# kobejean/nerf-qa

Hardware: AMD Instinct MI355X
Metric: DISTS frame-pairs/s (higher is better)
Workload: dtype f16

## Files before the change

nerf_qa_amd/csrc/nqa_conv.hip:

```cpp

#include "nqa_common.h"
#include "nqa_regw.h"

namespace nqa {

template <typename P>
__global__ __launch_bounds__(256) void conv1_1_kernel(const float *__restrict__ x, const float *__restrict__ w,
                                                      const float *__restrict__ bias,
                                                      typename P::T *__restrict__ out, int H, int W) {
  typedef typename P::T T;
  constexpr int HC = 128 / (int)sizeof(T);
  constexpr int PITCH = 128 + 16;
  __shared__ __attribute__((aligned(16))) char tile[256 * PITCH];
  const int HW = H * W;
  const int tid = threadIdx.x;
  const int pix0 = blockIdx.x * 256, pix = pix0 + tid;
  const int n = blockIdx.y;
  const bool live = pix < HW;
  const int py = live ? pix / W : 0, px = live ? pix - py * W : 0;
  float in[27];
  const float *xi = x + (size_t)n * 3 * HW;
#pragma unroll
  for (int ky = 0; ky < 3; ++ky) {
#pragma unroll
// ... 19 lines not shown
      f32x2 acc2[8];
#pragma unroll
      for (int j = 0; j < 8; ++j) acc2[j] = *reinterpret_cast<const f32x2 *>(bias + c0 + 2 * j);
#pragma unroll
      for (int k = 0; k < 27; ++k) {
#pragma unroll
        for (int j = 0; j < 8; ++j)
          acc2[j] = in[k] * *reinterpret_cast<const f32x2 *>(w + k * 64 + c0 + 2 * j) + acc2[j];
      }
      float acc[16];
#pragma unroll
      for (int j = 0; j < 16; ++j) acc[j] = acc2[j >> 1][j & 1];
      T *row = reinterpret_cast<T *>(tile + tid * PITCH) + g * 16;
      if constexpr (P::SPLIT) {
#pragma unroll
        for (int j = 0; j < 16; j += 4)
          store_split4(reinterpret_cast<char *>(row), j, fmaxf(acc[j], 0.f), fmaxf(acc[j + 1], 0.f),
                       fmaxf(acc[j + 2], 0.f), fmaxf(acc[j + 3], 0.f));
      } else if constexpr (sizeof(T) == 4) {
#pragma unroll
        for (int j = 0; j < 16; j += 4) {
          f32x4 v = {fmaxf(acc[j], 0.f), fmaxf(acc[j + 1], 0.f), fmaxf(acc[j + 2], 0.f), fmaxf(acc[j + 3], 0.f)};
          *reinterpret_cast<f32x4 *>(row + j) = v;
        }
      } else {
        typedef __attribute__((ext_vector_type(8))) T t8;
#pragma unroll
        for (int j = 0; j < 16; j += 8) {
          t8 v;
#pragma unroll
          for (int e = 0; e < 8; ++e) v[e] = P::from_f(fmaxf(acc[j + e], 0.f));
          *reinterpret_cast<t8 *>(row + j) = v;
        }
      }
    }
    __syncthreads();
#pragma unroll
    for (int r = 0; r < 8; ++r) {
      const int i = r * 256 + tid, p = i >> 3, ch = i & 7;
      if (p < npix)
        *reinterpret_cast<u32x4 *>(o + (size_t)p * 64 * sizeof(T) + half * 128 + ch * 16) =
            *reinterpret_cast<const u32x4 *>(tile + p * PITCH + ch * 16);
    }
    if (half + 1 < 64 / HC) __syncthreads();
  }
}


#ifdef NQA_STAMPS
__device__ unsigned long long g_stamps[8];
__device__ inline unsigned long long stamp() {
  unsigned long long t;
  __builtin_amdgcn_sched_barrier(0);
  asm volatile("s_memtime %0\n\ts_waitcnt lgkmcnt(0)" : "=s"(t)::"memory");
  __builtin_amdgcn_sched_barrier(0);
  return t;
}
#define NQA_STAMP(var) const unsigned long long var = stamp()
#define NQA_STAMP_ADD(seg, a, b) seg_sum[seg] += (b) - (a)
#else
#define NQA_STAMP(var)
#define NQA_STAMP_ADD(seg, a, b)
#endif

template <int WAVES_N, int WAVES_M, int WN_T, int WM_T, int TW, bool PAD8 = false>
struct ConvGeom {
  static constexpr int THREADS = 64 * WAVES_N * WAVES_M;
  static constexpr int BN = WAVES_N * WN_T * 32;
  static constexpr int NSUB = BN / 64;
  static constexpr int MP = WAVES_M * WM_T * 32;
  static constexpr int TH = MP / TW;
  static constexpr int HW_ = TW + 2, HH_ = TH + 2;
  static constexpr int HP = PAD8 ? (HW_ + 7) / 8 * 8 : HW_;
  static constexpr int NQ = HP * HH_;
  static constexpr int A_ITEMS = NQ * 4;
  static constexpr int A_ITEMS_PAD = (A_ITEMS + 63) / 64 * 64;
  static constexpr int A_BYTES = A_ITEMS_PAD * 16;
  static constexpr int A_ROUNDS = (A_ITEMS_PAD + THREADS - 1) / THREADS;
  static constexpr int SUB_STAGE_ITEMS = 3 * 64 * 4;
  static constexpr int W_ITEMS = NSUB * SUB_STAGE_ITEMS;
  static constexpr int W_BYTES = W_ITEMS * 16;
  static constexpr int W_ROUNDS = W_ITEMS / THREADS;
  static constexpr int LDS_BYTES = 2 * (A_BYTES + W_BYTES);
  static_assert(BN % 64 == 0 && W_ITEMS % THREADS == 0 && MP % TW == 0, "bad conv geometry");
};
static_assert(ConvGeom<2, 4, 4, 2, 32, true>::LDS_BYTES == 149504 && ConvGeom<2, 4, 4, 2, 16, true>::LDS_BYTES == 153600 &&
                  ConvGeom<2, 4, 2, 4, 32, true>::LDS_BYTES <= 163840,
              "8-wave M16 tiles: LDS budget");
static_assert(ConvGeom<2, 2, 2, 2, 32, true>::LDS_BYTES == 79872 && ConvGeom<2, 2, 2, 2, 16, true>::LDS_BYTES == 79872 &&
                  2 * 79872 <= 163840,
              "4-wave M16 tiles must keep two blocks per CU");

template <typename P, int WAVES_N, int WAVES_M, int WN_T, int WM_T, int TW, bool M16, int NTERM = 1, bool LOACC = false>
__device__ __forceinline__ void conv3x3_igemm_tile(
    const typename P::T *in, const char *wpk, const float *bias, typename P::T *out, int H, int W, int Cin, int Cout,
    int out_split, float floor_v, const int n, const int x0, const int y0, const int ct, char *const smem) {
#if defined(__HIP_DEVICE_COMPILE__)
  typedef typename P::T T;
  typedef ConvGeom<WAVES_N, WAVES_M, WN_T, WM_T, TW, M16> G;

  const int tid = threadIdx.x, lane = tid & 63;
  const int wave = __builtin_amdgcn_readfirstlane(tid >> 6);
  const int l31 = lane & 31, h = lane >> 5;
#if !defined(NQA_PRIO_SPLIT)
#define NQA_PRIO_SPLIT 2
#endif
  if (NQA_PRIO_SPLIT && M16 && WAVES_N * WAVES_M == 8 && wave >= 4) __builtin_amdgcn_s_setprio(NQA_PRIO_SPLIT);
  const int wn = wave % WAVES_N, wm = wave / WAVES_N;
  const int nCC = Cin / P::KC;
  const int S = nCC * 3 * NTERM;

  unsigned a_goff[G::A_ROUNDS];
#pragma unroll
  for (int r = 0; r < G::A_ROUNDS; ++r) {
    const int i = r * G::THREADS + tid;
    const int q = i >> 2, c = (i & 3) ^ lds_swz<M16>(q);
    const int hy = q / G::HP, hx = q - hy * G::HP;
    const int gy = y0 - 1 + hy, gx = x0 - 1 + hx;
    const bool ok = i < G::A_ITEMS && hx < G::HW_ && (unsigned)gy < (unsigned)H && (unsigned)gx < (unsigned)W;
    a_goff[r] = ok ? (unsigned)(((gy * W + gx) * Cin + c * P::CPC) * (int)sizeof(T)) : kOOB;
    if (!ok && i < G::A_ITEMS_PAD) {
      const u32x4 z = {0u, 0u, 0u, 0u};
      *reinterpret_cast<u32x4 *>(smem + i * 16) = z;
      *reinterpret_cast<u32x4 *>(smem + G::A_BYTES + i * 16) = z;
    }
  }
  const unsigned img_bytes = (unsigned)H * (unsigned)W * (unsigned)Cin * (unsigned)sizeof(T);
  const __amdgpu_buffer_rsrc_t a_rsrc = __builtin_amdgcn_make_buffer_rsrc(
      const_cast<T *>(in + (size_t)n * H * W * Cin), 0, img_bytes, 0x00020000);
  const unsigned sub_stride = (unsigned)nCC * 9u * 64u * 64u * (unsigned)NTERM;
  const __amdgpu_buffer_rsrc_t w_rsrc = __builtin_amdgcn_make_buffer_rsrc(
      const_cast<char *>(wpk + (size_t)ct * G::NSUB * sub_stride), 0, G::NSUB * sub_stride, 0x00020000);
  unsigned w_goff[G::W_ROUNDS];
#pragma unroll
  for (int r = 0; r < G::W_ROUNDS; ++r) {
    const int i = r * G::THREADS + tid;
    w_goff[r] = (unsigned)(i / G::SUB_STAGE_ITEMS) * sub_stride + (unsigned)(i % G::SUB_STAGE_ITEMS) * 16u;
  }
  const int wave_base = wave * 64 * 16;

  auto issue = [&](int s, int cc, bool first) {
#ifndef NQA_ABLATE_NO_DMA
    char *wdst = smem + 2 * G::A_BYTES + (s & 1) * G::W_BYTES + wave_base;
#pragma unroll
    for (int r = 0; r < G::W_ROUNDS; ++r)
      __builtin_amdgcn_raw_ptr_buffer_load_lds(w_rsrc, (lds_void_t *)(wdst + r * G::THREADS * 16), 16, w_goff[r],
                                               s * (G::SUB_STAGE_ITEMS * 16), 0, 0);
    if (first) {
      char *adst = smem + (cc & 1) * G::A_BYTES + wave_base;
#pragma unroll
      for (int r = 0; r < G::A_ROUNDS; ++r) {
        if (r * G::THREADS + wave * 64 < G::A_ITEMS_PAD)
          __builtin_amdgcn_raw_ptr_buffer_load_lds(a_rsrc, (lds_void_t *)(adst + r * G::THREADS * 16), 16, a_goff[r],
                                                   cc * 64, 0, 0);
      }
    }
#endif
  };
  auto dma_wait = [] { asm volatile("s_waitcnt vmcnt(0)" ::: "memory"); };

  int w_base[WN_T], w_sw[WN_T];
#pragma unroll
  for (int i = 0; i < WN_T; ++i) {
    const int cib = (wn * WN_T + i) * 32 + l31;
    const int r64 = cib & 63;
    w_base[i] = 2 * G::A_BYTES + (cib >> 6) * (G::SUB_STAGE_ITEMS * 16) + r64 * 64;
    w_sw[i] = (r64 >> 2) & 3;
  }
  int q0[WM_T];
#pragma unroll
  for (int j = 0; j < WM_T; ++j) {
    const int m = (wm * WM_T + j) * 32 + l31;
    const int ty = m / TW, tx = m - ty * TW;
    q0[j] = ty * G::HW_ + tx;
  }

  f32x16 acc[WN_T][WM_T];
#pragma unroll
  for (int i = 0; i < WN_T; ++i)
#pragma unroll
    for (int j = 0; j < WM_T; ++j)
#pragma unroll
      for (int r = 0; r < 16; ++r) acc[i][j][r] = 0.f;
  static_assert(!LOACC || (P::SPLIT && !M16), "LOACC: the split-f16 products only");
  f32x16 acc_lo[LOACC ? WN_T : 1][LOACC ? WM_T : 1];
  if constexpr (LOACC) {
#pragma unroll
    for (int i = 0; i < WN_T; ++i)
#pragma unroll
      for (int j = 0; j < WM_T; ++j)
#pragma unroll
        for (int r = 0; r < 16; ++r) acc_lo[i][j][r] = 0.f;
  }
  const int l15 = lane & 15, c4 = lane >> 4;
  int w16_base = 0, a16_base[3] = {0, 0, 0};
  auto w16_off = [](int i) { return (i >> 2) * (G::SUB_STAGE_ITEMS * 16) + (i & 3) * 1024; };
  auto a16_off = [](int j) { return ((j * 16 / TW) * G::HP + j * 16 % TW) * 64; };
  f32x4 acc16[2 * WN_T][2 * WM_T];
  if constexpr (M16) {
    static_assert(WN_T % 2 == 0 && (TW == 16 || TW == 32) && G::HP % 8 == 0 && (WM_T * 32) % TW == 0,
                  "the M16 loop's constant fragment offsets");
    static_assert(((2 * WM_T - 1) * 16 / TW * G::HP + 16) * 64 < 65536 &&
                      ((2 * WN_T - 1) >> 2) * (G::SUB_STAGE_ITEMS * 16) + 3 * 1024 + 2 * 4096 < 65536,
                  "an M16 fragment offset does not fit a ds_read immediate");
    w16_base = 2 * G::A_BYTES + wn * (WN_T / 2) * (G::SUB_STAGE_ITEMS * 16) + l15 * 64 + ((c4 ^ lds_swz<true>(l15)) << 4);
    const int qb = (wm * WM_T * 32 / TW) * G::HP + l15;
#pragma unroll
    for (int kx = 0; kx < 3; ++kx) a16_base[kx] = (qb + kx) * 64 + ((c4 ^ lds_swz<true>(qb + kx)) << 4);
#pragma unroll
    for (int i = 0; i < 2 * WN_T; ++i)
#pragma unroll
      for (int j = 0; j < 2 * WM_T; ++j) acc16[i][j] = (f32x4){0.f, 0.f, 0.f, 0.f};
  }

#ifdef NQA_STAMPS
  unsigned long long seg_sum[4] = {0, 0, 0, 0};
#endif
  issue(0, 0, true);
  for (int s = 0, cc = 0, sub = 0; s < S; ++s) {
    const int ky = sub / NTERM;
    const int sub_next = sub + 1 == 3 * NTERM ? 0 : sub + 1, cc_next = sub_next ? cc : cc + 1;
    NQA_STAMP(t0);
    dma_wait();
    NQA_STAMP(t1);
    __syncthreads();
    NQA_STAMP(t2);
    if (s + 1 < S) issue(s + 1, cc_next, sub_next == 0);
    NQA_STAMP(t3);
    NQA_STAMP_ADD(0, t0, t1);
    NQA_STAMP_ADD(1, t1, t2);
    NQA_STAMP_ADD(2, t2, t3);
    const char *abuf = smem + (cc & 1) * G::A_BYTES;
    const char *wbuf = smem + (s & 1) * G::W_BYTES;
    auto load_frags = [&](int t, u32x4(&af)[WN_T], u32x4(&bf)[WM_T]) {
      const int kx = t >> 1, ch = 2 * (t & 1) + h;
#pragma unroll
      for (int i = 0; i < WN_T; ++i)
        af[i] = *reinterpret_cast<const u32x4 *>(wbuf + w_base[i] + kx * 4096 + ((ch ^ w_sw[i]) << 4));
#pragma unroll
      for (int j = 0; j < WM_T; ++j) {
        const int q = q0[j] + ky * G::HW_ + kx;
        bf[j] = *reinterpret_cast<const u32x4 *>(abuf + q * 64 + ((ch ^ ((q >> 2) & 3)) << 4));
      }
    };
    auto mma_all = [&](const u32x4(&af)[WN_T], const u32x4(&bf)[WM_T]) {
#ifndef NQA_ABLATE_NO_MFMA
#pragma unroll
      for (int i = 0; i < WN_T; ++i)
#pragma unroll
        for (int j = 0; j < WM_T; ++j) acc[i][j] = P::mma(af[i], bf[j], acc[i][j]);
#else
#pragma unroll
      for (int i = 0; i < WN_T; ++i) asm volatile("" ::"v"(af[i]));
#pragma unroll
      for (int j = 0; j < WM_T; ++j) asm volatile("" ::"v"(bf[j]));
#endif
    };
    if constexpr (M16) {
      u32x4 af[2][WN_T], bf[2][2 * WM_T];
      const int a_stage = (cc & 1) * G::A_BYTES + ky * (G::HP * 64);
      const char *const wst = smem + (w16_base + (s & 1) * G::W_BYTES);
      const char *const ast[3] = {smem + (a16_base[0] + a_stage), smem + (a16_base[1] + a_stage),
                                  smem + (a16_base[2] + a_stage)};
      auto load16 = [&](int t) {
        const int kx = t >> 1, half = t & 1;
#pragma unroll
        for (int i = 0; i < WN_T; ++i)
          af[t & 1][i] = *reinterpret_cast<const u32x4 *>(wst + (w16_off(half * WN_T + i) + kx * 4096));
        if (half == 0) {
#pragma unroll
          for (int j = 0; j < 2 * WM_T; ++j) bf[kx & 1][j] = *reinterpret_cast<const u32x4 *>(ast[kx] + a16_off(j));
        }
      };
      auto mma16 = [&](int t) {
        const int kx = t >> 1, half = t & 1;
#pragma unroll
        for (int i = 0; i < WN_T; ++i)
#pragma unroll
          for (int j = 0; j < 2 * WM_T; ++j) {
            f32x4 &c = acc16[half * WN_T + i][j];
            c = P::mma16(af[t & 1][i], bf[kx & 1][j], c);
          }
      };
      load16(0);
#pragma unroll
      for (int t = 0; t < 6; ++t) {
        if (t + 1 < 6) load16(t + 1);
        __builtin_amdgcn_sched_barrier(0);
        mma16(t);
        __builtin_amdgcn_sched_barrier(0);
      }
    } else if constexpr (P::SPLIT) {
      auto load_split = [&](int kx, u32x4(&ah)[WN_T], u32x4(&al)[WN_T], u32x4(&bh)[WM_T], u32x4(&bl)[WM_T]) {
#pragma unroll
        for (int i = 0; i < WN_T; ++i) {
          const char *row = wbuf + w_base[i] + kx * 4096;
          ah[i] = *reinterpret_cast<const u32x4 *>(row + ((h ^ w_sw[i]) << 4));
          al[i] = *reinterpret_cast<const u32x4 *>(row + (((2 + h) ^ w_sw[i]) << 4));
        }
#pragma unroll
        for (int j = 0; j < WM_T; ++j) {
          const int q = q0[j] + ky * G::HW_ + kx, sw = (q >> 2) & 3;
          bh[j] = *reinterpret_cast<const u32x4 *>(abuf + q * 64 + ((h ^ sw) << 4));
          bl[j] = *reinterpret_cast<const u32x4 *>(abuf + q * 64 + (((2 + h) ^ sw) << 4));
        }
      };
      auto mma_split = [&](const u32x4(&ah)[WN_T], const u32x4(&al)[WN_T], const u32x4(&bh)[WM_T],
                           const u32x4(&bl)[WM_T]) {
#pragma unroll
        for (int term = 0; term < 3; ++term)
#pragma unroll
          for (int i = 0; i < WN_T; ++i)
#pragma unroll
            for (int j = 0; j < WM_T; ++j) {
              f32x16 &c = (LOACC && term < 2) ? acc_lo[LOACC ? i : 0][LOACC ? j : 0] : acc[i][j];
              c = __builtin_amdgcn_mfma_f32_32x32x16_f16(__builtin_bit_cast(f16x8, term == 0 ? al[i] : ah[i]),
                                                         __builtin_bit_cast(f16x8, term == 1 ? bl[j] : bh[j]), c, 0, 0, 0);
            }
      };
      u32x4 ahA[WN_T], alA[WN_T], bhA[WM_T], blA[WM_T], ahB[WN_T], alB[WN_T], bhB[WM_T], blB[WM_T];
      load_split(0, ahA, alA, bhA, blA);
      load_split(1, ahB, alB, bhB, blB);
      __builtin_amdgcn_sched_barrier(0);
      mma_split(ahA, alA, bhA, blA);
      __builtin_amdgcn_sched_barrier(0);
      load_split(2, ahA, alA, bhA, blA);
      __builtin_amdgcn_sched_barrier(0);
      mma_split(ahB, alB, bhB, blB);
      __builtin_amdgcn_sched_barrier(0);
      mma_split(ahA, alA, bhA, blA);
      __builtin_amdgcn_sched_barrier(0);
    } else {
    u32x4 afA[WN_T], bfA[WM_T], afB[WN_T], bfB[WM_T];
    load_frags(0, afA, bfA);
#pragma unroll
    for (int t = 0; t < 6; t += 2) {
      load_frags(t + 1, afB, bfB);
      __builtin_amdgcn_sched_barrier(0);
      mma_all(afA, bfA);
      __builtin_amdgcn_sched_barrier(0);
      if (t + 2 < 6) load_frags(t + 2, afA, bfA);
      __builtin_amdgcn_sched_barrier(0);
      mma_all(afB, bfB);
      __builtin_amdgcn_sched_barrier(0);
    }
    }
    NQA_STAMP(t4);
    NQA_STAMP_ADD(3, t3, t4);
    cc = cc_next;
    sub = sub_next;
  }
#ifdef NQA_STAMPS
  if (lane == 0) {
    for (int i = 0; i < 4; ++i) atomicAdd(&g_stamps[i], seg_sum[i]);
    atomicAdd(&g_stamps[4], (unsigned long long)S);
  }
#endif

  if constexpr (LOACC) {
#pragma unroll
    for (int i = 0; i < WN_T; ++i)
#pragma unroll
      for (int j = 0; j < WM_T; ++j) acc[i][j] += acc_lo[i][j];
  }
  constexpr int RB = G::BN * (int)sizeof(T), NCH = RB / 16, SWZ = NCH >= 16 ? 15 : NCH - 1;
  constexpr int ROWS = WAVES_M * 32;
  static_assert(ROWS * RB <= G::LDS_BYTES, "epilogue tile does not fit the stage buffers");
  char *const obase = reinterpret_cast<char *>(out) + (size_t)ct * RB;
  const size_t rec = (size_t)Cout * sizeof(T);
  const float winv = (P::SPLIT || NTERM == 2) ? bias[Cout] : 1.f;
  constexpr int NBQ = M16 ? 2 * WN_T : 4 * WN_T;
  f32x4 bq[NBQ];
#pragma unroll
  for (int q = 0; q < NBQ; ++q) {
    const int cl = M16 ? wn * WN_T * 32 + q * 16 + 4 * c4 : (wn * WN_T + (q >> 2)) * 32 + 8 * (q & 3) + 4 * h;
    bq[q] = *reinterpret_cast<const f32x4 *>(bias + ct * G::BN + cl);
  }
  auto stage_piece = [&](int row, int cl, const f32x4 &b4_pre, float a0, float a1, float a2, float a3) {
    char *const rbase = smem + row * RB;
    const int sw = row & SWZ;
#ifdef NQA_EPI_BIAS_INLINE
    const f32x4 b4 = *reinterpret_cast<const f32x4 *>(bias + ct * G::BN + cl);
    (void)b4_pre;
#else
    const f32x4 &b4 = b4_pre;
#endif
    if constexpr (P::SPLIT || NTERM == 2) {
      a0 *= winv;
      a1 *= winv;
      a2 *= winv;
      a3 *= winv;
    }
    const float v[4] = {fmaxf(a0 + b4[0], floor_v), fmaxf(a1 + b4[1], floor_v), fmaxf(a2 + b4[2], floor_v),
                        fmaxf(a3 + b4[3], floor_v)};
    if constexpr (sizeof(T) == 4) {
      if (P::SPLIT && out_split) {
        typedef __attribute__((ext_vector_type(4))) _Float16 h4;
        const h4 hi = {(_Float16)v[0], (_Float16)v[1], (_Float16)v[2], (_Float16)v[3]};
        const h4 lo = {(_Float16)(v[0] - (float)hi[0]), (_Float16)(v[1] - (float)hi[1]),
                       (_Float16)(v[2] - (float)hi[2]), (_Float16)(v[3] - (float)hi[3])};
        const int off = (cl >> 4) * 64 + ((cl >> 3) & 1) * 16 + (cl & 7) * 2;
        *reinterpret_cast<h4 *>(rbase + ((((off >> 4)) ^ sw) << 4) + (off & 15)) = hi;
        *reinterpret_cast<h4 *>(rbase + ((((off >> 4) + 2) ^ sw) << 4) + (off & 15)) = lo;
      } else {
        const f32x4 s4 = {v[0], v[1], v[2], v[3]};
        *reinterpret_cast<f32x4 *>(rbase + (((cl >> 2) ^ sw) << 4)) = s4;
      }
    } else {
      typedef __attribute__((ext_vector_type(4))) T t4;
      const t4 s4 = {P::from_f(v[0]), P::from_f(v[1]), P::from_f(v[2]), P::from_f(v[3])};
      *reinterpret_cast<t4 *>(rbase + (((cl >> 3) ^ sw) << 4) + (cl & 4) * 2) = s4;
    }
  };
#pragma unroll
  for (int j = 0; j < WM_T; ++j) {
    __syncthreads();
    if constexpr (M16) {
#pragma unroll
      for (int jj = 0; jj < 2; ++jj)
#pragma unroll
        for (int i = 0; i < 2 * WN_T; ++i) {
          const f32x4 &c = acc16[i][2 * j + jj];
          stage_piece(wm * 32 + jj * 16 + l15, wn * WN_T * 32 + i * 16 + 4 * c4, bq[i], c[0], c[1], c[2], c[3]);
        }
    } else {
#pragma unroll
      for (int i = 0; i < WN_T; ++i)
#pragma unroll
        for (int g = 0; g < 4; ++g)
          stage_piece(wm * 32 + l31, (wn * WN_T + i) * 32 + 8 * g + 4 * h, bq[M16 ? 0 : 4 * i + g], acc[i][j][4 * g],
                      acc[i][j][4 * g + 1], acc[i][j][4 * g + 2], acc[i][j][4 * g + 3]);
    }
    __syncthreads();
#pragma unroll 2
    for (int idx = tid; idx < ROWS * NCH; idx += G::THREADS) {
      const int row = idx / NCH, k = idx - row * NCH;
      const int m = ((row >> 5) * WM_T + j) * 32 + (row & 31);
      const int ty = m / TW, tx = m - ty * TW;
      const int gy = y0 + ty, gx = x0 + tx;
      if (gy < H && gx < W)
        *reinterpret_cast<u32x4 *>(obase + ((size_t)(n * H + gy) * W + gx) * rec + k * 16) =
            *reinterpret_cast<const u32x4 *>(smem + row * RB + ((k ^ (row & SWZ)) << 4));
    }
  }
#endif
}

__device__ __forceinline__ int xcd_tile_order(int id, int nb) {
  const int qq = nb >> 3, rr = nb & 7, xcd = id & 7, local = id >> 3;
  return (xcd < rr ? xcd * (qq + 1) : rr * (qq + 1) + (xcd - rr) * qq) + local;
}

template <typename P, int WAVES_N, int WAVES_M, int WN_T, int WM_T, int TW, bool M16, int NTERM = 1, bool LOACC = false>
__global__ __launch_bounds__(64 * WAVES_N * WAVES_M) void conv3x3_igemm_kernel(
    const typename P::T *__restrict__ in, const char *__restrict__ wpk, const float *__restrict__ bias,
    typename P::T *__restrict__ out, int H, int W, int Cin, int Cout, int tiles_x, int out_split, float floor_v) {
  typedef ConvGeom<WAVES_N, WAVES_M, WN_T, WM_T, TW, M16> G;
  extern __shared__ __attribute__((aligned(16))) char smem[];
  const int tile_id = xcd_tile_order(blockIdx.x, gridDim.x);
  const int bx = tile_id % tiles_x, by = tile_id / tiles_x;
  conv3x3_igemm_tile<P, WAVES_N, WAVES_M, WN_T, WM_T, TW, M16, NTERM, LOACC>(
      in, wpk, bias, out, H, W, Cin, Cout, out_split, floor_v, blockIdx.y, bx * TW, by * G::TH, blockIdx.z, smem);
}

template <typename P, int WAVES_N, int WAVES_M, int WN_T, int WM_T, bool M16, int NTERM = 1>
__global__ __launch_bounds__(64 * WAVES_N * WAVES_M) void conv3x3_igemm_mixed_kernel(
    const typename P::T *__restrict__ in, const char *__restrict__ wpk, const float *__restrict__ bias,
    typename P::T *__restrict__ out, int H, int W, int Cin, int Cout, int N, int main_tx, int main_tiles, int n_main,
    int edge_ty, int out_split, float floor_v) {
  extern __shared__ __attribute__((aligned(16))) char smem[];
  const int b = blockIdx.x;
  if (b < n_main) {
    typedef ConvGeom<WAVES_N, WAVES_M, WN_T, WM_T, 32, M16> G;
    const int g = xcd_tile_order(b, n_main);
    const int slab = g / main_tiles, tile_id = g - slab * main_tiles;
    const int bx = tile_id % main_tx, by = tile_id / main_tx;
    conv3x3_igemm_tile<P, WAVES_N, WAVES_M, WN_T, WM_T, 32, M16, NTERM>(
        in, wpk, bias, out, H, W, Cin, Cout, out_split, floor_v, slab % N, bx * 32, by * G::TH, slab / N, smem);
  } else {
    typedef ConvGeom<WAVES_N, WAVES_M, WN_T, WM_T, 16, M16> G;
    const int e = b - n_main;
    const int slab = e / edge_ty, by = e - slab * edge_ty;
    conv3x3_igemm_tile<P, WAVES_N, WAVES_M, WN_T, WM_T, 16, M16, NTERM>(
        in, wpk, bias, out, H, W, Cin, Cout, out_split, floor_v, slab % N, main_tx * 32, by * G::TH, slab / N, smem);
  }
}

template <typename P, int NCG, int NTERM = 1>
__global__ __launch_bounds__(512) void conv3x3_regw_kernel(const typename P::T *__restrict__ in,
                                                           const char *__restrict__ wreg,
                                                           const float *__restrict__ bias,
                                                           typename P::T *__restrict__ out, int H, int W, int tiles_x,
                                                           int tiles_y, int total_tiles) {
#if defined(__HIP_DEVICE_COMPILE__)
  typedef typename P::T T;
  constexpr int COUT = 32 * NCG, TH = 8, TW = 32, HWD = TW + 2, NQ = (TH + 2) * HWD;
  constexpr int CW = 32 / NTERM, NG = COUT / CW;
  constexpr int CH_ITEMS = 1536, CH_BYTES = CH_ITEMS * 16, SLOT = 2 * CH_BYTES;
  constexpr int NPIECE = 6;
  constexpr int RW = NG;
  constexpr int GPP = 2;
  constexpr int NPASS = 2 * RW / GPP;
  constexpr int NSTORE = (2 / NTERM) * GPP * NPASS;
  static_assert((NCG == 2 || NCG == 4) && (NTERM == 1 || NTERM == 2) && NG <= 8, "64 or 128 output channels");
  extern __shared__ __attribute__((aligned(16))) char smem[];
  const int tid = threadIdx.x, lane = tid & 63;
  const int wave = __builtin_amdgcn_readfirstlane(tid >> 6);
  const int l15 = lane & 15, c4 = lane >> 4;
  const int cg = wave % NG, ph = wave / NG;

  const TileRun run(total_tiles);
  const int my_tiles = run.count;
  if (my_tiles == 0) return;
  auto tile_coords = [&](int it, int &n, int &x0, int &y0) { run.coords<TH, TW>(it, tiles_x, tiles_y, n, x0, y0); };

  u32x4 wf[2][18];
#pragma unroll
  for (int i = 0; i < 2; ++i)
#pragma unroll
    for (int ks = 0; ks < 18; ++ks)
      wf[i][ks] = *reinterpret_cast<const u32x4 *>(wreg + ((((size_t)cg * 2 + i) * 18 + ks) * 64 + lane) * 16);
  float bia[2][4];
#pragma unroll
  for (int i = 0; i < 2; ++i)
#pragma unroll
    for (int e = 0; e < 4; ++e) bia[i][e] = bias[NTERM == 2 ? cg * 16 + 4 * c4 + e : cg * 32 + i * 16 + 4 * c4 + e];
  const float winv = NTERM == 2 ? bias[COUT] : 1.f;
// ... 1322 lines not shown
      }
    };
    auto mma_all = [&](const u32x4(&af)[WN_T], const u32x4(&bf)[WM_T]) {
#pragma unroll
      for (int i = 0; i < WN_T; ++i)
#pragma unroll
        for (int j = 0; j < WM_T; ++j) acc[i][j] = P::mma(af[i], bf[j], acc[i][j]);
    };
    u32x4 afA[WN_T], bfA[WM_T], afB[WN_T], bfB[WM_T];
    load_frags(0, afA, bfA);
#pragma unroll
    for (int t = 0; t < 6; t += 2) {
      load_frags(t + 1, afB, bfB);
      __builtin_amdgcn_sched_barrier(0);
      mma_all(afA, bfA);
      __builtin_amdgcn_sched_barrier(0);
      if (t + 2 < 6) load_frags(t + 2, afA, bfA);
      __builtin_amdgcn_sched_barrier(0);
      mma_all(afB, bfB);
      __builtin_amdgcn_sched_barrier(0);
    }
  }

  constexpr int RB = 64 * (int)sizeof(T), NCH = RB / 16, SWZ = NCH - 1, ROWS = 4 * 32;
  const size_t rec = (size_t)64 * sizeof(T);
  char *const obase = reinterpret_cast<char *>(out);
#pragma unroll
  for (int j = 0; j < WM_T; ++j) {
    __syncthreads();
    {
      const int row = wm * 32 + l31;
      char *const rbase = smem + row * RB;
      const int sw = row & SWZ;
#pragma unroll
      for (int i = 0; i < WN_T; ++i)
#pragma unroll
        for (int g = 0; g < 4; ++g) {
          const int cl = i * 32 + 8 * g + 4 * h;
          const f32x4 b4 = *reinterpret_cast<const f32x4 *>(bias2 + cl);
          typedef __attribute__((ext_vector_type(4))) T t4;
          t4 s4;
#pragma unroll
          for (int e = 0; e < 4; ++e) s4[e] = P::from_f(fmaxf(acc[i][j][4 * g + e] + b4[e], 0.f));
          *reinterpret_cast<t4 *>(rbase + (((cl >> 3) ^ sw) << 4) + (cl & 4) * 2) = s4;
        }
    }
    __syncthreads();
#pragma unroll 2
    for (int idx = tid; idx < ROWS * NCH; idx += G::THREADS) {
      const int row = idx / NCH, k = idx - row * NCH;
      const int m = ((row >> 5) * WM_T + j) * 32 + (row & 31);
      const int ty = m / TW, tx = m - ty * TW;
      const int gy = y0 + ty, gx = x0 + tx;
      if (gy < H && gx < W)
        *reinterpret_cast<u32x4 *>(obase + ((size_t)(n * H + gy) * W + gx) * rec + k * 16) =
            *reinterpret_cast<const u32x4 *>(smem + row * RB + ((k ^ (row & SWZ)) << 4));
    }
  }
#endif
}

#ifdef NQA_STAMPS
extern "C" int nqa_debug_stamps(unsigned long long *out8, int reset) {
  if (hipMemcpyFromSymbol(out8, HIP_SYMBOL(g_stamps), 8 * sizeof(unsigned long long)) != hipSuccess) return -1;
  if (reset) {
    unsigned long long z[8] = {0};
    if (hipMemcpyToSymbol(HIP_SYMBOL(g_stamps), z, sizeof(z)) != hipSuccess) return -1;
  }
  return 0;
}
#endif

template <typename P>
static int launch_conv1_1(const float *x, int n, int H, int W, const char *packed, void *out, hipStream_t st,
                          int blob_prec = P::ID) {
  const float *w = reinterpret_cast<const float *>(packed + layer_offset(0, blob_prec));
  const float *b = reinterpret_cast<const float *>(packed + layer_bias_offset(0, blob_prec));
  dim3 grid(cdiv(H * W, 256), n);
  TimedLaunch t(NQA_K_CONV1, st);
  conv1_1_kernel<P><<<grid, 256, 0, st>>>(x, w, b, reinterpret_cast<typename P::T *>(out), H, W);
  return check_launch("conv1_1");
}

template <typename P, int WAVES_N, int WAVES_M, int WN_T, int WM_T, int TW, bool M16 = (sizeof(typename P::T) == 2), int NTERM = 1,
          bool LOACC = false>
static int launch_igemm(const void *in, int n, int H, int W, int cin, int cout, const char *wpk, const float *bias,
                        void *out, int out_split, hipStream_t st, float floor_v = 0.f) {
  typedef ConvGeom<WAVES_N, WAVES_M, WN_T, WM_T, TW, M16> G;
  if (const int rc = lds_limit<conv3x3_igemm_kernel<P, WAVES_N, WAVES_M, WN_T, WM_T, TW, M16, NTERM, LOACC>>(G::LDS_BYTES, "conv3x3_igemm")) return rc;
  const int tiles_x = cdiv(W, TW), tiles_y = cdiv(H, G::TH);
  dim3 grid(tiles_x * tiles_y, n, cout / G::BN);
  TimedLaunch t(NQA_K_CONV, st);
  conv3x3_igemm_kernel<P, WAVES_N, WAVES_M, WN_T, WM_T, TW, M16, NTERM, LOACC><<<grid, G::THREADS, G::LDS_BYTES, st>>>(
      reinterpret_cast<const typename P::T *>(in), wpk, bias, reinterpret_cast<typename P::T *>(out), H, W, cin, cout,
      tiles_x, out_split, floor_v);
  return check_launch("conv3x3_igemm");
}

static bool use_mixed_grid(int n, int H, int W, int ctiles, int MP, int blocks_per_cu) {
  const int rem = W % 32;
  const int edge_grid = tuning().edge_grid;
  if (edge_grid == 1 || rem < 1 || rem > 16 || W < 32) return false;
  if (edge_grid == 2) return true;
  const long slots = (long)num_cus(nullptr) * blocks_per_cu;
  if (slots <= 0) return false;
  const long per = (long)n * ctiles;
  const long plain = (long)cdiv(W, 32) * cdiv(H, MP / 32) * per;
  const long mixed = ((long)(W / 32) * cdiv(H, MP / 32) + cdiv(H, MP / 16)) * per;
  return (mixed + slots - 1) / slots < (plain + slots - 1) / slots;
}

template <typename P, int WAVES_N, int WAVES_M, int WN_T, int WM_T, bool M16 = (sizeof(typename P::T) == 2), int NTERM = 1>
static int launch_igemm_mixed(const void *in, int n, int H, int W, int cin, int cout, const char *wpk, const float *bias,
                              void *out, int out_split, hipStream_t st) {
  typedef ConvGeom<WAVES_N, WAVES_M, WN_T, WM_T, 32, M16> GM;
  typedef ConvGeom<WAVES_N, WAVES_M, WN_T, WM_T, 16, M16> GE;
  constexpr int LDS = GM::LDS_BYTES > GE::LDS_BYTES ? GM::LDS_BYTES : GE::LDS_BYTES;
  if (const int rc = lds_limit<conv3x3_igemm_mixed_kernel<P, WAVES_N, WAVES_M, WN_T, WM_T, M16, NTERM>>(LDS, "conv3x3_igemm_mixed")) return rc;
  const int main_tx = W / 32, main_tiles = main_tx * cdiv(H, GM::TH), edge_ty = cdiv(H, GE::TH);
  const long slabs = (long)n * (cout / GM::BN);
  const long n_main = main_tiles * slabs, n_total = n_main + edge_ty * slabs;
  if (main_tx < 1 || n_total > 0x7fffffffL) {
    set_error("conv3x3_igemm_mixed: %d x %d x %d images do not fit the mixed grid", n, H, W);
    return NQA_E_SHAPE;
  }
  TimedLaunch t(NQA_K_CONV, st);
  conv3x3_igemm_mixed_kernel<P, WAVES_N, WAVES_M, WN_T, WM_T, M16, NTERM><<<dim3((unsigned)n_total), GM::THREADS, LDS, st>>>(
      reinterpret_cast<const typename P::T *>(in), wpk, bias, reinterpret_cast<typename P::T *>(out), H, W, cin, cout, n,
      main_tx, main_tiles, (int)n_main, edge_ty, out_split, 0.f);
  ++tuning().mixed_launches;
  return check_launch("conv3x3_igemm_mixed");
}

template <typename P, int NCG = 4, int NTERM = 1>
static int launch_regw(const void *in, int n, int H, int W, int layer, const char *packed, void *out, hipStream_t st,
                       int blob_prec = P::ID) {
  constexpr int LDS = 3 * 2 * 1536 * 16;
  if (const int rc = lds_limit<conv3x3_regw_kernel<P, NCG, NTERM>>(LDS, "conv3x3_regw")) return rc;
  const int cus = num_cus("conv3x3_regw");
  if (!cus) return NQA_E_LAUNCH;
  const int tiles_x = cdiv(W, 32), tiles_y = cdiv(H, 8), total = n * tiles_x * tiles_y;
  const int grid = total < cus ? total : cus;
  const float *bias = reinterpret_cast<const float *>(packed + layer_bias_offset(layer, blob_prec));
  TimedLaunch t(NQA_K_CONV, st);
  conv3x3_regw_kernel<P, NCG, NTERM><<<grid, 512, LDS, st>>>(reinterpret_cast<const typename P::T *>(in),
                                                             packed + regw_offset(layer, blob_prec), bias,
                                                             reinterpret_cast<typename P::T *>(out), H, W, tiles_x,
                                                             tiles_y, total);
  return check_launch("conv3x3_regw");
}

static int launch_regw_split(const void *in, int n, int H, int W, int layer, const char *packed, void *out, hipStream_t st) {
  constexpr int LDS = 2 * 2 * 204 * 160;
  if (const int rc = lds_limit<conv3x3_regw_split_kernel>(LDS, "conv3x3_regw_split")) return rc;
  const int cus = num_cus("conv3x3_regw_split");
  if (!cus) return NQA_E_LAUNCH;
  const int cout = kConvs[layer].cout, nh = cout / 64;
  const int tiles_x = cdiv(W, 32), tiles_y = cdiv(H, 4), total = n * tiles_x * tiles_y;
  int streams = cus / (8 * nh);
  if (streams > cdiv(total, 8)) streams = cdiv(total, 8);
  if (streams < 1) streams = 1;
  const int grid = 8 * nh * streams;
  const float *bias = reinterpret_cast<const float *>(packed + layer_bias_offset(layer, NQA_PREC_F32S));
  TimedLaunch t(NQA_K_CONV, st);
  conv3x3_regw_split_kernel<<<grid, 512, LDS, st>>>(static_cast<const char *>(in), packed + regw_offset(layer, NQA_PREC_F32S),
                                                    bias, static_cast<char *>(out), H, W, tiles_x, tiles_y, total, cout);
  return check_launch("conv3x3_regw_split");
}

template <typename P, int NTERM = 1>
static int launch_regw128(const void *in, int n, int H, int W, int layer, const char *packed, void *out, hipStream_t st,
                          int blob_prec = P::ID) {
  constexpr int LDS = 2 * 4 * 1024 * 16, PF = 3;
  if (const int rc = lds_limit<conv3x3_regw128_kernel<P, PF, NTERM>>(LDS, "conv3x3_regw128")) return rc;
  const int cus = num_cus("conv3x3_regw128");
  if (!cus) return NQA_E_LAUNCH;
  const int cout = kConvs[layer].cout, nct = cout / (128 / NTERM);
  const int tiles_x = cdiv(W, 32), tiles_y = cdiv(H, 4), total = n * tiles_x * tiles_y * nct;
  int grid = total < cus ? total : cus;
  while (nct > 1 && grid > 8 * nct && ((grid + 7) / 8) % nct) grid -= 8;
  const float *bias = reinterpret_cast<const float *>(packed + layer_bias_offset(layer, blob_prec));
  TimedLaunch t(NQA_K_CONV, st);
  conv3x3_regw128_kernel<P, PF, NTERM><<<grid, 256, LDS, st>>>(reinterpret_cast<const typename P::T *>(in),
                                                               packed + regw_offset(layer, blob_prec), bias,
                                                               reinterpret_cast<typename P::T *>(out), H, W, cout,
                                                               tiles_x, tiles_y, total);
  return check_launch("conv3x3_regw128");
}

template <typename P, int NTERM>
static int launch_conv(const void *in, int n, int H, int W, int layer, const char *packed, int blob_prec, void *out,
                       hipStream_t st) {
  static_assert(NTERM == 1 || (NTERM == 2 && P::ID == NQA_PREC_F16), "two-term weights exist for the f16 kernels only");
  constexpr bool B16 = sizeof(typename P::T) == 2;
  const Tuning &tn = tuning();
  const ConvSpec &cs = kConvs[layer];
  const char *wpk = packed + layer_offset(layer, blob_prec);
  const float *bias = reinterpret_cast<const float *>(packed + layer_bias_offset(layer, blob_prec));
  const bool narrow = W <= 16;
  const int out_split = P::SPLIT && !cs.last;
// ... 212 lines not shown
```

Measured before the change: 450.6.

## Overlap first weight DMA with setup and streamline conv epilogue copy-out

Issues the first weight-stage DMA before computing activation offsets, so the prologue address math overlaps the load. Bias is copied once into a small LDS region and read from there in the epilogue. The copy-out now uses precomputed swizzled LDS offsets and buffer stores that rely on out-of-range masking instead of per-element bounds checks. When all passes fit in LDS, it stages them with a single barrier pair instead of two per pass. This adds a few hundred bytes of LDS per block and a 32-bit output offset limit, which is now checked on the host.

Result: no change. 451.7 (median of 6 runs) (+0.3%).

```diff
diff --git a/nerf_qa_amd/csrc/nqa_conv.hip b/nerf_qa_amd/csrc/nqa_conv.hip
--- a/nerf_qa_amd/csrc/nqa_conv.hip
+++ b/nerf_qa_amd/csrc/nqa_conv.hip
@@ -125,13 +125,16 @@
   static constexpr int W_BYTES = W_ITEMS * 16;
   static constexpr int W_ROUNDS = W_ITEMS / THREADS;
   static constexpr int LDS_BYTES = 2 * (A_BYTES + W_BYTES);
+  static constexpr int BIAS_OFF = LDS_BYTES, BIAS_BYTES = BN * 4;
+  static constexpr int LDS_TOTAL = LDS_BYTES + BIAS_BYTES;
   static_assert(BN % 64 == 0 && W_ITEMS % THREADS == 0 && MP % TW == 0, "bad conv geometry");
+  static_assert(LDS_TOTAL <= 163840, "the stage buffers and the bias copy do not fit a CU's LDS");
 };
 static_assert(ConvGeom<2, 4, 4, 2, 32, true>::LDS_BYTES == 149504 && ConvGeom<2, 4, 4, 2, 16, true>::LDS_BYTES == 153600 &&
                   ConvGeom<2, 4, 2, 4, 32, true>::LDS_BYTES <= 163840,
               "8-wave M16 tiles: LDS budget");
 static_assert(ConvGeom<2, 2, 2, 2, 32, true>::LDS_BYTES == 79872 && ConvGeom<2, 2, 2, 2, 16, true>::LDS_BYTES == 79872 &&
-                  2 * 79872 <= 163840,
+                  2 * ConvGeom<2, 2, 2, 2, 32, true>::LDS_TOTAL <= 163840,
               "4-wave M16 tiles must keep two blocks per CU");
 
 template <typename P, int WAVES_N, int WAVES_M, int WN_T, int WM_T, int TW, bool M16, int NTERM = 1, bool LOACC = false>
@@ -142,6 +145,7 @@
   typedef typename P::T T;
   typedef ConvGeom<WAVES_N, WAVES_M, WN_T, WM_T, TW, M16> G;
 
+  NQA_STAMP(t_entry);
   const int tid = threadIdx.x, lane = tid & 63;
   const int wave = __builtin_amdgcn_readfirstlane(tid >> 6);
   const int l31 = lane & 31, h = lane >> 5;
@@ -152,6 +156,28 @@
   const int wn = wave % WAVES_N, wm = wave / WAVES_N;
   const int nCC = Cin / P::KC;
   const int S = nCC * 3 * NTERM;
+
+  const int wave_base = wave * 64 * 16;
+  const unsigned sub_stride = (unsigned)nCC * 9u * 64u * 64u * (unsigned)NTERM;
+  const __amdgpu_buffer_rsrc_t w_rsrc = __builtin_amdgcn_make_buffer_rsrc(
+      const_cast<char *>(wpk + (size_t)ct * G::NSUB * sub_stride), 0, G::NSUB * sub_stride, 0x00020000);
+  unsigned w_goff[G::W_ROUNDS];
+#pragma unroll
+  for (int r = 0; r < G::W_ROUNDS; ++r) {
+    const int i = r * G::THREADS + tid;
+    w_goff[r] = (unsigned)(i / G::SUB_STAGE_ITEMS) * sub_stride + (unsigned)(i % G::SUB_STAGE_ITEMS) * 16u;
+  }
+  auto issue_w = [&](int s) {
+#ifndef NQA_ABLATE_NO_DMA
+    char *wdst = smem + 2 * G::A_BYTES + (s & 1) * G::W_BYTES + wave_base;
+#pragma unroll
+    for (int r = 0; r < G::W_ROUNDS; ++r)
+      __builtin_amdgcn_raw_ptr_buffer_load_lds(w_rsrc, (lds_void_t *)(wdst + r * G::THREADS * 16), 16, w_goff[r],
+                                               s * (G::SUB_STAGE_ITEMS * 16), 0, 0);
+#endif
+  };
+  issue_w(0);
+  NQA_STAMP(t_first_dma);
 
   unsigned a_goff[G::A_ROUNDS];
 #pragma unroll
@@ -171,36 +197,45 @@
   const unsigned img_bytes = (unsigned)H * (unsigned)W * (unsigned)Cin * (unsigned)sizeof(T);
   const __amdgpu_buffer_rsrc_t a_rsrc = __builtin_amdgcn_make_buffer_rsrc(
       const_cast<T *>(in + (size_t)n * H * W * Cin), 0, img_bytes, 0x00020000);
-  const unsigned sub_stride = (unsigned)nCC * 9u * 64u * 64u * (unsigned)NTERM;
-  const __amdgpu_buffer_rsrc_t w_rsrc = __builtin_amdgcn_make_buffer_rsrc(
-      const_cast<char *>(wpk + (size_t)ct * G::NSUB * sub_stride), 0, G::NSUB * sub_stride, 0x00020000);
-  unsigned w_goff[G::W_ROUNDS];
-#pragma unroll
-  for (int r = 0; r < G::W_ROUNDS; ++r) {
-    const int i = r * G::THREADS + tid;
-    w_goff[r] = (unsigned)(i / G::SUB_STAGE_ITEMS) * sub_stride + (unsigned)(i % G::SUB_STAGE_ITEMS) * 16u;
-  }
-  const int wave_base = wave * 64 * 16;
-
+  auto issue_a = [&](int cc) {
+#ifndef NQA_ABLATE_NO_DMA
+    char *adst = smem + (cc & 1) * G::A_BYTES + wave_base;
+#pragma unroll
+    for (int r = 0; r < G::A_ROUNDS; ++r) {
+      if (r * G::THREADS + wave * 64 < G::A_ITEMS_PAD)
+        __builtin_amdgcn_raw_ptr_buffer_load_lds(a_rsrc, (lds_void_t *)(adst + r * G::THREADS * 16), 16, a_goff[r],
+                                                 cc * 64, 0, 0);
+    }
+#endif
+  };
+  issue_a(0);
   auto issue = [&](int s, int cc, bool first) {
-#ifndef NQA_ABLATE_NO_DMA
-    char *wdst = smem + 2 * G::A_BYTES + (s & 1) * G::W_BYTES + wave_base;
-#pragma unroll
-    for (int r = 0; r < G::W_ROUNDS; ++r)
-      __builtin_amdgcn_raw_ptr_buffer_load_lds(w_rsrc, (lds_void_t *)(wdst + r * G::THREADS * 16), 16, w_goff[r],
-                                               s * (G::SUB_STAGE_ITEMS * 16), 0, 0);
-    if (first) {
-      char *adst = smem + (cc & 1) * G::A_BYTES + wave_base;
-#pragma unroll
-      for (int r = 0; r < G::A_ROUNDS; ++r) {
-        if (r * G::THREADS + wave * 64 < G::A_ITEMS_PAD)
-          __builtin_amdgcn_raw_ptr_buffer_load_lds(a_rsrc, (lds_void_t *)(adst + r * G::THREADS * 16), 16, a_goff[r],
-                                                   cc * 64, 0, 0);
-      }
-    }
-#endif
+    issue_w(s);
+    if (first) issue_a(cc);
   };
   auto dma_wait = [] { asm volatile("s_waitcnt vmcnt(0)" ::: "memory"); };
+
+  if (tid < G::BN / 4)
+    *reinterpret_cast<f32x4 *>(smem + G::BIAS_OFF + tid * 16) = *reinterpret_cast<const f32x4 *>(bias + ct * G::BN + tid * 4);
+
+  constexpr int RB = G::BN * (int)sizeof(T), NCH = RB / 16, SWZ = NCH >= 16 ? 15 : NCH - 1;
+  constexpr int ROWS = WAVES_M * 32, PASS_BYTES = ROWS * RB;
+  constexpr int RSTEP = G::THREADS / NCH, NIT = ROWS / RSTEP;
+  constexpr int NPH = RSTEP > SWZ ? 1 : (SWZ + 1) / RSTEP, NTX = RSTEP >= TW ? 1 : TW / RSTEP;
+  static_assert((NCH & (NCH - 1)) == 0 && (RSTEP & (RSTEP - 1)) == 0 && RSTEP * NCH == G::THREADS && RSTEP <= 32 &&
+                    ROWS % RSTEP == 0 && (TW == 16 || TW == 32),
+                "the copy-out's constant item steps");
+  const unsigned rec32 = (unsigned)Cout * (unsigned)sizeof(T);
+  const int co_r0 = tid / NCH, co_k = tid % NCH;
+  int co_lds[NPH];
+#pragma unroll
+  for (int p = 0; p < NPH; ++p) co_lds[p] = co_r0 * RB + ((co_k ^ (co_r0 & SWZ) ^ (p * RSTEP)) << 4);
+  const int co_tx = x0 + (co_r0 & (TW - 1)), co_ty = y0 + co_r0 / TW;
+  const int co_yrem = H - co_ty;
+  unsigned co_goff[NTX];
+#pragma unroll
+  for (int t = 0; t < NTX; ++t)
+    co_goff[t] = co_tx + t * RSTEP < W ? (unsigned)(co_ty * W + co_tx) * rec32 + (unsigned)(ct * RB + co_k * 16) : kOOB;
 
   int w_base[WN_T], w_sw[WN_T];
 #pragma unroll
@@ -257,9 +292,8 @@
   }
 
 #ifdef NQA_STAMPS
-  unsigned long long seg_sum[4] = {0, 0, 0, 0};
-#endif
-  issue(0, 0, true);
+  unsigned long long seg_sum[4] = {0, 0, 0, 0}, t_first_barrier = 0;
+#endif
   for (int s = 0, cc = 0, sub = 0; s < S; ++s) {
     const int ky = sub / NTERM;
     const int sub_next = sub + 1 == 3 * NTERM ? 0 : sub + 1, cc_next = sub_next ? cc : cc + 1;
@@ -273,6 +307,9 @@
     NQA_STAMP_ADD(0, t0, t1);
     NQA_STAMP_ADD(1, t1, t2);
     NQA_STAMP_ADD(2, t2, t3);
+#ifdef NQA_STAMPS
+    if (s == 0) t_first_barrier = t2;
+#endif
     const char *abuf = smem + (cc & 1) * G::A_BYTES;
     const char *wbuf = smem + (s & 1) * G::W_BYTES;
     auto load_frags = [&](int t, u32x4(&af)[WN_T], u32x4(&bf)[WM_T]) {
@@ -393,12 +430,7 @@
     cc = cc_next;
     sub = sub_next;
   }
-#ifdef NQA_STAMPS
-  if (lane == 0) {
-    for (int i = 0; i < 4; ++i) atomicAdd(&g_stamps[i], seg_sum[i]);
-    atomicAdd(&g_stamps[4], (unsigned long long)S);
-  }
-#endif
+  NQA_STAMP(t_loop_end);
 
   if constexpr (LOACC) {
 #pragma unroll
@@ -406,28 +438,18 @@
 #pragma unroll
       for (int j = 0; j < WM_T; ++j) acc[i][j] += acc_lo[i][j];
   }
-  constexpr int RB = G::BN * (int)sizeof(T), NCH = RB / 16, SWZ = NCH >= 16 ? 15 : NCH - 1;
-  constexpr int ROWS = WAVES_M * 32;
-  static_assert(ROWS * RB <= G::LDS_BYTES, "epilogue tile does not fit the stage buffers");
-  char *const obase = reinterpret_cast<char *>(out) + (size_t)ct * RB;
-  const size_t rec = (size_t)Cout * sizeof(T);
+  static_assert(PASS_BYTES <= G::LDS_BYTES, "epilogue tile does not fit the stage buffers");
   const float winv = (P::SPLIT || NTERM == 2) ? bias[Cout] : 1.f;
   constexpr int NBQ = M16 ? 2 * WN_T : 4 * WN_T;
   f32x4 bq[NBQ];
 #pragma unroll
   for (int q = 0; q < NBQ; ++q) {
     const int cl = M16 ? wn * WN_T * 32 + q * 16 + 4 * c4 : (wn * WN_T + (q >> 2)) * 32 + 8 * (q & 3) + 4 * h;
-    bq[q] = *reinterpret_cast<const f32x4 *>(bias + ct * G::BN + cl);
-  }
-  auto stage_piece = [&](int row, int cl, const f32x4 &b4_pre, float a0, float a1, float a2, float a3) {
-    char *const rbase = smem + row * RB;
+    bq[q] = *reinterpret_cast<const f32x4 *>(smem + G::BIAS_OFF + cl * 4);
+  }
+  auto stage_piece = [&](char *const tile, int row, int cl, const f32x4 &b4, float a0, float a1, float a2, float a3) {
+    char *const rbase = tile + row * RB;
     const int sw = row & SWZ;
-#ifdef NQA_EPI_BIAS_INLINE
-    const f32x4 b4 = *reinterpret_cast<const f32x4 *>(bias + ct * G::BN + cl);
-    (void)b4_pre;
-#else
-    const f32x4 &b4 = b4_pre;
-#endif
     if constexpr (P::SPLIT || NTERM == 2) {
       a0 *= winv;
       a1 *= winv;
@@ -455,37 +477,72 @@
       *reinterpret_cast<t4 *>(rbase + (((cl >> 3) ^ sw) << 4) + (cl & 4) * 2) = s4;
     }
   };
-#pragma unroll
-  for (int j = 0; j < WM_T; ++j) {
-    __syncthreads();
+  auto stage_pass = [&](int j, char *const tile) {
     if constexpr (M16) {
 #pragma unroll
       for (int jj = 0; jj < 2; ++jj)
 #pragma unroll
         for (int i = 0; i < 2 * WN_T; ++i) {
           const f32x4 &c = acc16[i][2 * j + jj];
-          stage_piece(wm * 32 + jj * 16 + l15, wn * WN_T * 32 + i * 16 + 4 * c4, bq[i], c[0], c[1], c[2], c[3]);
+          stage_piece(tile, wm * 32 + jj * 16 + l15, wn * WN_T * 32 + i * 16 + 4 * c4, bq[i], c[0], c[1], c[2], c[3]);
         }
     } else {
 #pragma unroll
       for (int i = 0; i < WN_T; ++i)
 #pragma unroll
         for (int g = 0; g < 4; ++g)
-          stage_piece(wm * 32 + l31, (wn * WN_T + i) * 32 + 8 * g + 4 * h, bq[M16 ? 0 : 4 * i + g], acc[i][j][4 * g],
-                      acc[i][j][4 * g + 1], acc[i][j][4 * g + 2], acc[i][j][4 * g + 3]);
-    }
+          stage_piece(tile, wm * 32 + l31, (wn * WN_T + i) * 32 + 8 * g + 4 * h, bq[M16 ? 0 : 4 * i + g],
+                      acc[i][j][4 * g], acc[i][j][4 * g + 1], acc[i][j][4 * g + 2], acc[i][j][4 * g + 3]);
+    }
+  };
+  const __amdgpu_buffer_rsrc_t o_rsrc = __builtin_amdgcn_make_buffer_rsrc(
+      out + (size_t)n * H * W * Cout, 0, (unsigned)H * (unsigned)W * rec32, 0x00020000);
+  auto copy_pass = [&](int j, const char *const tile) {
+    constexpr int CHUNK = NIT < 8 ? NIT : 8;
+    static_assert(NIT % CHUNK == 0, "copy-out chunks");
+#pragma unroll
+    for (int i0 = 0; i0 < NIT; i0 += CHUNK) {
+      u32x4 v[CHUNK];
+#pragma unroll
+      for (int e = 0; e < CHUNK; ++e)
+        v[e] = *reinterpret_cast<const u32x4 *>(tile + co_lds[(i0 + e) % NPH] + (i0 + e) * (RSTEP * RB));
+#pragma unroll
+      for (int e = 0; e < CHUNK; ++e) {
+        const int c = RSTEP * (i0 + e), clo = c & 31, chi = c >> 5;
+        const int txc = clo & (TW - 1), tyc = (chi * WM_T + j) * (32 / TW) + clo / TW;
+        const unsigned voff =
+            (co_goff[txc / RSTEP] + (unsigned)(tyc * W + txc) * rec32) | ((unsigned)(co_yrem - 1 - tyc) & kOOB);
+        __builtin_amdgcn_raw_buffer_store_b128(v[e], o_rsrc, voff, 0, 0);
+      }
+    }
+  };
+  constexpr bool STAGE_ALL = WM_T * PASS_BYTES <= G::LDS_BYTES;
+  if constexpr (STAGE_ALL) {
     __syncthreads();
-#pragma unroll 2
-    for (int idx = tid; idx < ROWS * NCH; idx += G::THREADS) {
-      const int row = idx / NCH, k = idx - row * NCH;
-      const int m = ((row >> 5) * WM_T + j) * 32 + (row & 31);
-      const int ty = m / TW, tx = m - ty * TW;
-      const int gy = y0 + ty, gx = x0 + tx;
-      if (gy < H && gx < W)
-        *reinterpret_cast<u32x4 *>(obase + ((size_t)(n * H + gy) * W + gx) * rec + k * 16) =
-            *reinterpret_cast<const u32x4 *>(smem + row * RB + ((k ^ (row & SWZ)) << 4));
-    }
-  }
+#pragma unroll
+    for (int j = 0; j < WM_T; ++j) stage_pass(j, smem + j * PASS_BYTES);
+    __syncthreads();
+#pragma unroll
+    for (int j = 0; j < WM_T; ++j) copy_pass(j, smem + j * PASS_BYTES);
+  } else {
+#pragma unroll
+    for (int j = 0; j < WM_T; ++j) {
+      __syncthreads();
+      stage_pass(j, smem);
+      __syncthreads();
+      copy_pass(j, smem);
+    }
+  }
+#ifdef NQA_STAMPS
+  NQA_STAMP(t_exit);
+  if (lane == 0) {
+    for (int i = 0; i < 4; ++i) atomicAdd(&g_stamps[i], seg_sum[i]);
+    atomicAdd(&g_stamps[4], (unsigned long long)S);
+    atomicAdd(&g_stamps[5], t_first_dma - t_entry);
+    atomicAdd(&g_stamps[6], t_first_barrier - t_first_dma);
+    atomicAdd(&g_stamps[7], t_exit - t_loop_end);
+  }
+#endif
 #endif
 }
 
@@ -1974,16 +2031,26 @@
   return check_launch("conv1_1");
 }
 
+static int igemm_output_fits(const char *who, int H, int W, int cout, size_t elem_bytes) {
+  if ((long)H * W * cout * (long)elem_bytes >= (1L << 31)) {
+    set_error("%s: output map too large for 32-bit in-image byte offsets (H*W*%d channels*%d bytes >= 2^31)", who, cout,
+              (int)elem_bytes);
+    return NQA_E_SHAPE;
+  }
+  return 0;
+}
+
 template <typename P, int WAVES_N, int WAVES_M, int WN_T, int WM_T, int TW, bool M16 = (sizeof(typename P::T) == 2), int NTERM = 1,
           bool LOACC = false>
 static int launch_igemm(const void *in, int n, int H, int W, int cin, int cout, const char *wpk, const float *bias,
                         void *out, int out_split, hipStream_t st, float floor_v = 0.f) {
   typedef ConvGeom<WAVES_N, WAVES_M, WN_T, WM_T, TW, M16> G;
-  if (const int rc = lds_limit<conv3x3_igemm_kernel<P, WAVES_N, WAVES_M, WN_T, WM_T, TW, M16, NTERM, LOACC>>(G::LDS_BYTES, "conv3x3_igemm")) return rc;
+  if (const int rc = igemm_output_fits("conv3x3_igemm", H, W, cout, sizeof(typename P::T))) return rc;
+  if (const int rc = lds_limit<conv3x3_igemm_kernel<P, WAVES_N, WAVES_M, WN_T, WM_T, TW, M16, NTERM, LOACC>>(G::LDS_TOTAL, "conv3x3_igemm")) return rc;
   const int tiles_x = cdiv(W, TW), tiles_y = cdiv(H, G::TH);
   dim3 grid(tiles_x * tiles_y, n, cout / G::BN);
   TimedLaunch t(NQA_K_CONV, st);
-  conv3x3_igemm_kernel<P, WAVES_N, WAVES_M, WN_T, WM_T, TW, M16, NTERM, LOACC><<<grid, G::THREADS, G::LDS_BYTES, st>>>(
+  conv3x3_igemm_kernel<P, WAVES_N, WAVES_M, WN_T, WM_T, TW, M16, NTERM, LOACC><<<grid, G::THREADS, G::LDS_TOTAL, st>>>(
       reinterpret_cast<const typename P::T *>(in), wpk, bias, reinterpret_cast<typename P::T *>(out), H, W, cin, cout,
       tiles_x, out_split, floor_v);
   return check_launch("conv3x3_igemm");
@@ -2007,7 +2074,8 @@
                               void *out, int out_split, hipStream_t st) {
   typedef ConvGeom<WAVES_N, WAVES_M, WN_T, WM_T, 32, M16> GM;
   typedef ConvGeom<WAVES_N, WAVES_M, WN_T, WM_T, 16, M16> GE;
-  constexpr int LDS = GM::LDS_BYTES > GE::LDS_BYTES ? GM::LDS_BYTES : GE::LDS_BYTES;
+  constexpr int LDS = GM::LDS_TOTAL > GE::LDS_TOTAL ? GM::LDS_TOTAL : GE::LDS_TOTAL;
+  if (const int rc = igemm_output_fits("conv3x3_igemm_mixed", H, W, cout, sizeof(typename P::T))) return rc;
   if (const int rc = lds_limit<conv3x3_igemm_mixed_kernel<P, WAVES_N, WAVES_M, WN_T, WM_T, M16, NTERM>>(LDS, "conv3x3_igemm_mixed")) return rc;
   const int main_tx = W / 32, main_tiles = main_tx * cdiv(H, GM::TH), edge_ty = cdiv(H, GE::TH);
   const long slabs = (long)n * (cout / GM::BN);
```
